# duckdb/duckdb-vss

Hardware: AMD Instinct MI355X
Metric: queries/sec at recall@10, 10M×768 FLOAT top-10; index build rows/sec (higher is better)
Workload: dtype f32

## Files before the change

### duckdb-vss_amd/__init__.py

```python
import ctypes as C
import os
import subprocess

import numpy as np

HERE = os.path.dirname(os.path.abspath(__file__))
ROOT = os.path.dirname(HERE)
LIB_PATH = os.environ.get("VSS_LIBRARY") or os.path.join(HERE, "libvssgpu.so")
CSRC = os.path.join(HERE, "csrc")

METRICS = {"l2sq": 0, "cosine": 1, "ip": 2}
FUNCTIONS = {"array_distance": 0, "array_cosine_distance": 1, "array_negative_inner_product": 2}
FREE_KEY = np.iinfo(np.int64).max

HIPCC_FLAGS = ["--offload-arch=gfx950", "-O3", "-std=c++17", "-ffp-contract=off", "-fPIC", "-Wno-int-to-pointer-cast"]


TRANSLATION_UNITS = ["vss_engine.hip", "vss_exchange.hip", "kernels_l2sq.hip", "kernels_cosine.hip", "kernels_ip.hip"]


def build_library(force=False, extra_flags=(), out=None):
    out = out or os.path.join(HERE, "libvssgpu.so")
    srcs = [os.path.join(CSRC, f) for f in sorted(os.listdir(CSRC))]
    srcs.append(os.path.join(ROOT, "include", "vssgpu.h"))
# ... 34 lines not shown
    "vss_set_build_reorder": (_int, [_vp, _int]),
    "vss_set_option": (_int, [_vp, C.c_char_p, _i64]),
    "vss_search": (_int, [_vp, _vp, _u64, _u64, _vp, _vp]),
    "vss_search_batch": (_int, [_vp, _vp, _u64, _u64, _u64, _vp, _vp, _vp]),
    "vss_search_batch_device": (_int, [_vp, _vp, _u64, _u64, _u64, _vp, _vp, _vp]),
    "vss_search_batch_filtered": (_int, [_vp, _vp, _u64, _u64, _u64, _vp, _u64, _vp, _vp, _vp]),
    "vss_search_batch_filtered_device": (_int, [_vp, _vp, _u64, _u64, _u64, _vp, _u64, _vp, _vp, _vp]),
    "vss_search_batch_device_begin": (_int, [_vp, _int, _vp, _u64, _u64, _u64, _vp, _vp, _vp]),
    "vss_search_multi_device_begin": (_int, [_vp, _int, _u64, _vp, _u64, _u64, _u64, _vp, _vp, _vp]),
    "vss_search_batch_end": (_int, [_vp, _int]),
    "vss_search_exact_batch": (_int, [_vp, _vp, _u64, _u64, _vp, _vp, _vp]),
    "vss_search_exact_batch_device": (_int, [_vp, _vp, _u64, _u64, _vp, _vp, _vp]),
    "vss_last_search_stats": (_int, [_vp, _vp]),
    "vss_last_search_shape": (_int, [_vp, _vp]),
    "vss_last_search_prescore": (_int, [_vp, _vp]),
    "vss_last_search_query_stats": (_int, [_vp, _vp, _u64]),
    "vss_timing": (_int, [_vp, _vp, _int]),
    "vss_build_work": (_int, [_vp, _vp]),
    "vss_remove_batch": (_int, [_vp, _vp, _u64, _vp]),
    "vss_compact": (_int, [_vp]),
    "vss_compact_ex": (_int, [_vp, _int, _vp]),
    "vss_size": (_u64, [_vp]),
    "vss_nodes": (_u64, [_vp]),
    "vss_build_progress": (_int, [_vp, _vp, _vp]),
    "vss_capacity": (_u64, [_vp]),
    "vss_max_level": (_u64, [_vp]),
    "vss_memory_usage": (_u64, [_vp]),
    "vss_dimensions": (_u64, [_vp]),
    "vss_metric": (_int, [_vp]),
    "vss_level_stats": (_int, [_vp, _u64, _vp]),
# ... 207 lines not shown
    def last_search_stats(self):
        out = np.zeros(4, dtype=np.uint64)
        self._check(self.lib.vss_last_search_stats(self.h, _p(out)))
        return out

    def last_search_shape(self):
        out = np.zeros(8, dtype=np.uint32)
        self._check(self.lib.vss_last_search_shape(self.h, _p(out)))
        return out

    def last_search_prescore(self):
        out = np.zeros(4, dtype=np.uint64)
        self._check(self.lib.vss_last_search_prescore(self.h, _p(out)))
        return out

    def timing(self, reset=False):
        out = np.zeros(6, dtype=np.float64)
        self._check(self.lib.vss_timing(self.h, _p(out), int(reset)))
        return dict(search_kernel_ms=out[0], build_phase_a_ms=out[1], build_phase_b_ms=out[2], build_wall_ms=out[3],
                    build_batches=int(out[4]), build_retries=int(out[5]))

    def build_work(self):
        out = np.zeros(3, dtype=np.uint64)
        self._check(self.lib.vss_build_work(self.h, _p(out)))
        return dict(insert_distances=int(out[0]), insert_expansions=int(out[1]), link_distances=int(out[2]))

    def last_query_stats(self, nq):
        out = np.zeros((nq, 2), dtype=np.uint32)
        self._check(self.lib.vss_last_search_query_stats(self.h, _p(out), nq))
        return out
# ... 90 lines not shown
```

### duckdb-vss_amd/csrc/hnsw_kernels.h

```cpp
#pragma once
#include "wave_primitives.h"
#include "prescore_bound.h"
#include <type_traits>

namespace vss {

constexpr int64_t FREE_KEY = 0x7FFFFFFFFFFFFFFFll;

struct GraphView {
	RowSpace sp;
	uint32_t dim;
	uint32_t M, M0;
	uint32_t *links0;
	uint32_t *links_up;
	const uint32_t *upper_off;
	const int64_t *keys;
	uint32_t list_id_base;
	const unsigned long long *filter;
	uint64_t filter_bits;
	uint32_t twins;

	__device__ __forceinline__ bool admitted(uint32_t slot) const {
		const int64_t key = keys[slot];
		if (key == 0x7FFFFFFFFFFFFFFFll)
// ... 342 lines not shown
#define VSS_TRACE(sp, idx, expr)
#define VSS_TRACE_INC(sp, idx)
#endif
#ifndef VSS_WALKER_WAIT_SLEEP
#define VSS_WALKER_WAIT_SLEEP 1
#endif
#ifndef VSS_SCORER_IDLE_SLEEP
#define VSS_SCORER_IDLE_SLEEP 2
#endif
struct Mailbox {
	unsigned long long ticket;
	uint32_t done;
	uint32_t qa2_bits;
	uint32_t slots;
	uint32_t bound_bits;
	uint32_t pad[2];
};

struct PrescoreView {
	const uint32_t *codes;
	const RowCodeMeta *meta;
	unsigned long long *counters;
};
constexpr uint32_t PRESCORE_SLOTS = 16;
__host__ __device__ constexpr int prescore_claim_rows(int R) {
	return 4 * R;
}
__device__ __forceinline__ float code_to_float(uint32_t w, int k) {
	return (float)(int)(int8_t)(w >> (8 * k));
}
template <int MT, int NCH, int CR>
__device__ __forceinline__ unsigned long long prescore_codes(const RowSpace &sp, const PrescoreView &pv, uint32_t dim,
                                                             const float4 *q_lds, float qa2, const uint32_t *ids, int n,
// ... 147 lines not shown
				}
				VSS_LDS_ADD(lds_u32, done_or_scrap, cnt);
				worked = true;
				continue;
			}
		}
#endif
		const float qa2 = __uint_as_float(VSS_LDS_LOAD(lds_u32, &mb->qa2_bits));
		if constexpr (PRE) {
			if (pv->codes) {
				const float bound = __uint_as_float((uint32_t)uniform((int)VSS_LDS_LOAD(lds_u32, &mb->bound_bits)));
			if (bound < __builtin_inff()) {
					constexpr int CR = prescore_claim_rows(R);
					constexpr int SHIFT = CR == 16 ? 2 : CR == 8 ? 3 : 4;
					static_assert(CR == 16 || CR == 8 || CR == 4, "rows of codes per claim");
					unsigned long long left = prescore_codes<MT, NCH, CR>(sp, *pv, dim, q, qa2, ids + c, (int)cnt, bound, dist + c, pre_counts[1]);
					pre_counts[0] += cnt;
					while (left) {
						const int have = __popcll(left);
						if (have >= 3 && R >= 4)
							wave_distances_picked<MT, NCH, (R >= 4 ? 4 : 1)>(sp, q, qa2, ids + c, left, SHIFT, dist + c);
						else if (have >= 2)
							wave_distances_picked<MT, NCH, 2>(sp, q, qa2, ids + c, left, SHIFT, dist + c);
						else
							wave_distances_picked<MT, NCH, 1>(sp, q, qa2, ids + c, left, SHIFT, dist + c);
					}
					wave_sync();
					VSS_LDS_ADD_REL(lds_u32, done_or_scrap, cnt);
					VSS_TRACE_INC(sp, 29);
					worked = true;
					continue;
				}
// ... 21 lines not shown
constexpr uint32_t ENGINE_HEADER_BYTES = ENGINE_SCRAP_OFFSET + 64 * 8;

constexpr uint32_t POOL_SPIN_LIMIT = 1u << 26;

struct CrewBox {
	int n;
	float qa2;
	uint32_t walker;
	uint32_t on;
};
static_assert(sizeof(CrewBox) == 16 && sizeof(Mailbox) == 32, "engine LDS header layout");

template <int MT, int NCH, int R, bool PRE = false>
struct PoolScorer {
	static constexpr bool touches_rows = false, touches_lists = true, helpers_touch = false;
	Mailbox *mb;
	uint32_t *exit_flag;
	uint32_t *engine_error;
	uint32_t *walkers_left;
	uint32_t scorers;
	CrewBox *crew;
	uint32_t my_slot;
	uint32_t crew_ok;
	uint32_t no_requests;
	uint32_t touch_ok;
	uint32_t prescore_ok;
	mutable uint32_t crew_on = 0;
	mutable uint32_t level = 0;
	__device__ __forceinline__ void at_level(int l) const {
		level = (uint32_t)l;
	}

	__device__ __forceinline__ bool wants_requests() const {
		return !(crew_on && no_requests);
	}

	__device__ __forceinline__ bool latency_mode() const {
		return crew_on != 0 && touch_ok != 0;
	}
	__device__ __forceinline__ uint32_t active_walkers() const {
		const uint32_t active = (uint32_t)uniform((int)VSS_LDS_LOAD(lds_u32, walkers_left));
		return active ? active : 1u;
	}
	__device__ __forceinline__ void post(int buf, const RowSpace &sp, int n, float bound = __builtin_inff()) const {
		Mailbox *box = mb + buf;
		const uint32_t lg = 6u - sp.logG;
		const uint32_t x1 = ((uint32_t)n + (1u << lg) - 1u) >> lg, x2 = (x1 + 1u) >> 1;
		const uint32_t a = active_walkers();
		if (PRE && prescore_ok) {
			const bool filtered = bound < __builtin_inff() && a * x2 > scorers;
			VSS_LDS_STORE(lds_u32, &box->slots, a * x1 <= scorers ? 1u : a * x2 <= scorers ? 2u : filtered ? PRESCORE_SLOTS : (uint32_t)R);
			VSS_LDS_STORE(lds_u32, &box->bound_bits, __float_as_uint(filtered ? bound : __builtin_inff()));
		} else {
			VSS_LDS_STORE(lds_u32, &box->slots, a * x1 <= scorers ? 1u : a * x2 <= scorers ? 2u : (uint32_t)R);
		}
		VSS_LDS_STORE(lds_u32, &box->done, 0u);
		VSS_LDS_STORE_REL(lds_u64, &box->ticket, (unsigned long long)(uint32_t)n << 32);
		VSS_TRACE_INC(sp, 16);
		VSS_TRACE(sp, 17, (uint32_t)n);
	}
	__device__ __forceinline__ void wait(int buf, const RowSpace &sp, int n) const {
		Mailbox *box = mb + buf;
		uint32_t spins = 0;
		while (uniform((int)VSS_LDS_LOAD_ACQ(lds_u32, &box->done)) < n) {
			__builtin_amdgcn_s_sleep(VSS_WALKER_WAIT_SLEEP);
			if ((spins & 1023u) == 0) {
				VSS_TRACE(sp, 20, spins);
				VSS_TRACE(sp, 21, VSS_LDS_LOAD(lds_u32, &box->done));
			}
			if (++spins > POOL_SPIN_LIMIT || ((spins & 1023u) == 0 && uniform((int)VSS_LDS_LOAD(lds_u32, exit_flag)))) {
				if (lane_id() == 0) {
					VSS_LDS_STORE(lds_u32, exit_flag, 2u);
					__hip_atomic_store(engine_error, 1u, __ATOMIC_RELAXED, __HIP_MEMORY_SCOPE_SYSTEM);
				}
				__builtin_amdgcn_endpgm();
			}
		}
		wave_sync();
		VSS_TRACE_INC(sp, 18);
	}
	__device__ __forceinline__ void begin(int buf, const RowSpace &sp, float qa2, int n, float bound = __builtin_inff()) const {
		if (crew_ok && !crew_on && uniform((int)VSS_LDS_LOAD(lds_u32, walkers_left)) == 1) {
			crew_on = 1u;
#ifdef VSS_PHASE_TIMERS
			if (lane_id() < 3)
				reinterpret_cast<unsigned long long *>(reinterpret_cast<unsigned char *>(crew) - ENGINE_CREW_OFFSET + ENGINE_SCRAP_OFFSET)[lane_id()] = 0;
#endif
			VSS_LDS_STORE_REL(lds_u32, &crew->on, 1u);
		}
		if (crew_on) {
			if (lane_id() == 0) {
				crew->n = n;
				crew->qa2 = qa2;
				crew->walker = 2u * my_slot + (uint32_t)buf + (level << 8);
			}
			lds_barrier();
			return;
		}
		post(buf, sp, n, bound);
	}
	__device__ __forceinline__ void end(int buf, const RowSpace &sp, int n) const {
		if (crew_on)
			lds_barrier();
		else
			wait(buf, sp, n);
	}
	template <typename F>
	__device__ __forceinline__ void operator()(const WaveLds &lds, const RowSpace &sp, float qa2, int n, F before_loads
	                                           VSS_WC_ARG) const {
		if (n <= 0) {
			before_loads();
			return;
		}
		VSS_TICK(tp0);
		begin(0, sp, qa2, n);
		VSS_TICK(tpb);
		VSS_ACC(t_solo_passes, tp0, tpb);
		before_loads();
		VSS_TICK(tp1);
		end(0, sp, n);
		VSS_TICK(tp3);
		VSS_ACC(t_look, tp0, tp1);
		VSS_ACC(t_sync2, tp1, tp3);
	}
	__device__ __forceinline__ void dismiss_crew() const {
		if (lane_id() == 0)
			crew->n = -1;
		lds_barrier();
	}
};

template <int MT, bool AHEAD = false, class Scorer>
__device__ __forceinline__ uint32_t descend(const GraphView &gv, WaveLds &lds, float qa2, uint32_t closest,
                                            int begin_level, int end_level, const Scorer &score, WorkCounters &wc) {
	const int lane = lane_id();
	float closest_dist = wave_distance_one<MT>(gv.sp, lds.q, qa2, closest);
	wc.distances += 1;
	ListPrefetch below;
	int below_level = -1;
	const bool can_ahead = AHEAD && gv.M0 <= 64;
	for (int level = begin_level; level > end_level; --level) {
		bool changed;
		do {
			changed = false;
			const bool have_first = can_ahead && below.slot == closest && below_level == level;
			const int n = gather_neighbors<false>(gv, lds, closest, level, have_first, have_first ? below.masked() : EMPTY_SLOT);
			if constexpr (AHEAD)
				score.at_level(level);
			score(lds, gv.sp, qa2, n, [&] {
				if constexpr (AHEAD) {
					if (can_ahead && !(below.slot == closest && below_level == level - 1)) {
						below.slot = EMPTY_SLOT;
						below.request(gv, closest, level - 1);
						below_level = level - 1;
					}
				}
			} VSS_WC_PASS);
			wc.distances += n;
			wc.cycles += 1;
			for (int off = 0; off < n; off += 64) {
				const float d = (off + lane < n) ? lds.dist[off + lane] : __builtin_inff();
				float m = d;
				m = fminf(m, lane_xor<32>(m));
				m = fminf(m, lane_xor<16>(m));
				m = fminf(m, lane_xor<8>(m));
				m = fminf(m, lane_xor<4>(m));
				m = fminf(m, lane_xor<2>(m));
				m = fminf(m, lane_xor<1>(m));
				if (m < closest_dist) {
					const unsigned long long who = __ballot(d == m);
					closest_dist = m;
					closest = lds.ids[off + __builtin_ctzll(who)];
// ... 381 lines not shown
			have = L.first_two_unexpanded_entry(d1, s1, s2);
		} else {
			have = L.first_unexpanded_entry(d1, s1) >= 0 ? 1 : 0;
		}
		e_d = have > 0 ? d1 : __builtin_inff();
		e_s = have > 0 ? s1 : EMPTY_SLOT;
		if (!pool.wants_requests())
			return;
		if (have > 0)
			ahead.request(gv, s1, 0);
		if constexpr (PK > 1) {
			if (have > 1)
				ahead.request(gv, s2, 0);
		}
	};
	auto open_expansion = [&](uint32_t cs, int buf) -> int {
		VSS_TICK(tg0);
		uint32_t first_cells;
		const bool have_first = ahead.find(cs, first_cells);
		VSS_COUNT(t_slice, have_first ? 1u : 0u);
		lds.ids = sb.ids(buf);
		const int n = gather_neighbors<true>(gv, lds, cs, 0, have_first, first_cells);
		VSS_TICK(tg1);
		VSS_ACC(t_gather, tg0, tg1);
		if (n > 0)
			pool.begin(buf, gv.sp, qa2, n, L.size >= limit ? radius : __builtin_inff());
		VSS_TICK(tg2);
		VSS_ACC(t_solo_passes, tg1, tg2);
		return n;
	};
	auto accept = [&](int buf, int n) {
		const bool have = lane < n;
		const float d = have ? sb.dist(buf)[lane] : 0.f;
		const uint32_t id = have ? sb.ids(buf)[lane] : 0;
		const unsigned long long pass = __ballot(have && (L.size < limit || d < radius));
		L.accept(d, id, pass, radius);
	};

	int b = 0, n_cur = 0;
	for (;;) {
		if (n_cur == 0) {
			VSS_TICK(tk0);
			float cd;
			uint32_t cs;
			const int pos = L.first_unexpanded_entry(cd, cs);
			if (pos < 0)
				break;
			L.mark_expanded(pos);
			wc.cycles += 1;
			VSS_TICK(tk1);
			VSS_ACC(t_pick, tk0, tk1);
			n_cur = open_expansion(cs, b);
			if (n_cur < 0)
				return LEVEL_VISITED_OVERFLOW;
			request_ahead();
			continue;
		}
		VSS_TICK(tw0);
		pool.end(b, gv.sp, n_cur);
		VSS_TICK(tw1);
		VSS_ACC(t_sync2, tw0, tw1);
		wc.distances += n_cur;
		uint32_t next = EMPTY_SLOT;
		bool tie;
		{
			const bool have = lane < n_cur;
			const float d = have ? sb.dist(b)[lane] : 0.f;
			const uint32_t id = have ? sb.ids(b)[lane] : 0;
			const bool admitted = have && (L.size < limit || d < radius);
			float m = admitted ? d : __builtin_inff();
			m = fminf(m, lane_xor<32>(m));
			m = fminf(m, lane_xor<16>(m));
			m = fminf(m, lane_xor<8>(m));
			m = fminf(m, lane_xor<4>(m));
			m = fminf(m, lane_xor<2>(m));
			m = fminf(m, lane_xor<1>(m));
			const unsigned long long who = __ballot(admitted && !(d > m));
			const float ms = __int_as_float(uniform(__float_as_int(m)));
			tie = who && (__popcll(who) > 1 || !(__builtin_fabsf(ms) < __builtin_inff()) || ms == e_d);
			if (!tie)
				next = (who && ms < e_d) ? read_lane(id, __builtin_ctzll(who)) : e_s;
		}
		VSS_TICK(tw2);
		VSS_ACC(t_pick, tw1, tw2);
		if (tie) {
			accept(b, n_cur);
			n_cur = 0;
			VSS_TICK(tw3);
			VSS_ACC(t_accept, tw2, tw3);
			continue;
		}
		const int nb = 1 - b;
		int n_next = 0;
		if (next != EMPTY_SLOT) {
			wc.cycles += 1;
			n_next = open_expansion(next, nb);
			if (n_next < 0)
				return LEVEL_VISITED_OVERFLOW;
		}
		VSS_TICK(ta0);
		accept(b, n_cur);
		uint32_t first = EMPTY_SLOT;
		int pos;
		{
			float cd;
			uint32_t w = EMPTY_SLOT;
			pos = L.first_unexpanded_entry(cd, w);
			if (pos >= 0)
				first = w;
		}
		if (first != next) {
// ... 95 lines not shown
	float *out_d[MAX_COALESCED];
	uint32_t *out_count[MAX_COALESCED];
	uint32_t *out_stats;
	uint32_t *status;
	uint32_t *retry_hash;
	uint32_t retry_log2;
	uint32_t *global_hash;
	float *list_buf;
	uint32_t list_cap;
	uint32_t list_lds;
	float *cand_buf;
	uint32_t cand_cap;
	uint32_t visited_compact;
	unsigned long long *phase_ticks;
	PrescoreView prescore;
};

__host__ __device__ inline uint32_t align16(uint32_t x) {
	return (x + 15u) & ~15u;
}

__host__ __device__ inline uint32_t wave_lds_bytes(uint32_t hash_log2, uint32_t V, uint32_t list_cap_max,
                                                   uint32_t cand_cap, bool hash_in_lds = true) {
	uint32_t b = 0;
	if (hash_in_lds)
		b += align16((1u << hash_log2) * 4);
	b += align16(V * 16) * 2;
	b += align16(list_cap_max * 4) * 2;
	b += align16(cand_cap * 4) * 2;
	b += align16((list_cap_max + 1) * 4) * 2;
// ... 261 lines not shown
		*exit_flag = 0;
		*walkers_left = S;
		crew->n = 0, crew->qa2 = 0.f, crew->walker = 0, crew->on = 0;
		a.queue[a.queue_sel ^ 2u] = 0;
	}
	VSS_TRACE(a.gv.sp, 30, blockDim.x);
	VSS_TRACE(a.gv.sp, 31, S);
	if (lane == 0)
		smem[ENGINE_SIMD_OFFSET + wave] = (unsigned char)__builtin_amdgcn_s_getreg((1 << 11) | (4 << 6) | 4);
	if (threadIdx.x < ENGINE_BOXES) {
		boxes[threadIdx.x].ticket = 0;
		boxes[threadIdx.x].done = 0;
		boxes[threadIdx.x].qa2_bits = 0;
		boxes[threadIdx.x].slots = R;
		boxes[threadIdx.x].bound_bits = 0x7F800000u;
	}
	__syncthreads();
	constexpr bool PRE = NCH >= 2 && E >= 1 && E != LDS_LIST_E && E <= pipelined_max_regs(THREADS);

	if (wave >= S) {
		uint32_t pre_counts[2] = {0, 0};
		auto leave = [&] {
			if constexpr (PRE) {
				if (lane == 0 && pre_counts[0]) {
					atomicAdd(a.prescore.counters, (unsigned long long)pre_counts[0]);
					atomicAdd(a.prescore.counters + 1, (unsigned long long)pre_counts[1]);
				}
			}
		};
		for (;;) {
			bool worked = false;
			VSS_TRACE_INC(a.gv.sp, 24);
			for (uint32_t s = 0; s < 2 * S; ++s) {
				const unsigned long long t = VSS_LDS_LOAD(lds_u64, &boxes[s].ticket);
				if (uniform((int)((uint32_t)t < (uint32_t)(t >> 32)))) {
					const EngineSlot es =
					    engine_slot(smem, s >> 1, a.hash_log2, a.gv.sp.V, a.list_cap_max, hash_in_lds, a.stage_cap, list_cells);
					worked |= pool_score<MT, NCH, R, PRE>(&boxes[s], scrap, a.gv.sp, es.q, (s & 1) ? es.ids2 : es.ids,
					                                      (s & 1) ? es.dist2 : es.dist, &a.prescore, a.gv.dim, pre_counts);
				}
			}
// ... 14 lines not shown
	__builtin_amdgcn_s_setprio(2);
	const EngineSlot es = engine_slot(smem, wave, a.hash_log2, a.gv.sp.V, a.list_cap_max, hash_in_lds, a.stage_cap, list_cells);
	const size_t gslot = (size_t)blockIdx.x * S + wave;
	WaveLds lds;
	bind_visited(lds.visited, hash_in_lds ? es.hash : a.global_hash + (gslot << a.hash_log2), a.hash_log2);
	if constexpr (E == MAX_LIST_REGS) {
		if (a.visited_compact)
			bind_visited_compact(lds.visited, a.visited_compact);
	}
	lds.q = es.q, lds.ids = es.ids, lds.dist = es.dist;
	lds.q2 = nullptr, lds.kept_s = nullptr, lds.kept_d = nullptr;
	lds.cand_d = nullptr, lds.cand_s = nullptr;
	lds.touch_lines = a.touch_lines & TOUCH_LISTS;
	PoolScorer<MT, NCH, R, PRE> score {&boxes[2 * wave], exit_flag, a.engine_error, walkers_left, (blockDim.x >> 6) - S, crew, wave,
	                                   ((a.crew & CREW_ON) && !a.spec_active) ? 1u : 0u, (a.crew & CREW_NO_REQUESTS) ? 1u : 0u,
	                                   (a.crew & CREW_TOUCH) ? 1u : 0u, (PRE && a.prescore.codes) ? 1u : 0u};
	const SpecBuffers sb {es.ids, es.ids2, es.dist, es.dist2};
	CandQueue cq;
	cq.bind(a.cand_buf + gslot * 2 * a.cand_cap, reinterpret_cast<uint32_t *>(a.cand_buf + gslot * 2 * a.cand_cap) + a.cand_cap,
	        (int)a.cand_cap);
	typename std::conditional<E == LDS_LIST_E, LdsList,
	                          typename std::conditional<E == 0, MemList, WaveList<(E == 0 || E == LDS_LIST_E ? 1 : E)>>::type>::type L;
	if constexpr (E == 0)
		L.bind(a.list_buf + gslot * 2 * a.list_cap, reinterpret_cast<uint32_t *>(a.list_buf + gslot * 2 * a.list_cap) + a.list_cap);
	if constexpr (E == LDS_LIST_E)
		L.bind(es.list_d, es.list_s, es.list_tops);
	const int limit = a.ef > a.k ? a.ef : a.k;

	constexpr bool CAN_MOVE = E == MAX_LIST_REGS;
	if constexpr (CAN_MOVE) {
		if (a.retry_hash && hash_in_lds && es.stage_d) {
// ... 601 lines not shown
```

### duckdb-vss_amd/csrc/prescore_bound.h

```cpp
#pragma once
#include <math.h>
#include <stdint.h>

#if defined(__HIPCC__) || defined(__CUDACC__)
#define VSS_PRESCORE_HD __host__ __device__
#else
#define VSS_PRESCORE_HD
#endif

namespace vss {

struct RowCodeMeta {
	float scale;
	float err;
	float norm;
	uint32_t spare;
};

constexpr float PRESCORE_NO_BOUND = -INFINITY;

VSS_PRESCORE_HD inline double prescore_slack(uint32_t dim) {
	return ((double)dim + 64.0) * (1.0 / 2097152.0);
}

// ... 22 lines not shown
	} else {
		if (!(fabsf(t) < INFINITY))
			return PRESCORE_NO_BOUND;
		const double ub = scale * (double)t + qn * E;
		const double qr = qn * rn;
		if (metric == 1)
			lb = 1.0 - ub / qr - slack;
		else
			lb = 1.0 - ub - slack * qr - 0x1p-22 * (1.0 + qr);
	}
	if (!(lb == lb))
		return PRESCORE_NO_BOUND;
	return prescore_round_down(lb);
}

}
```

### duckdb-vss_amd/csrc/vss_engine.hip

```cpp
#include <hip/hip_runtime.h>

#include <algorithm>
#include <atomic>
#include <chrono>
#include <cmath>
#include <cstdarg>
#include <cstdio>
#include <cstdlib>
#include <cstring>
#include <condition_variable>
#include <mutex>
#include <shared_mutex>
#include <string>
#include <thread>
#include <vector>

#define VSS_ENGINE_TU
#include "../../include/vssgpu.h"
#include "launchers.h"
#include "host_logic.h"
#include "row_codes.h"

using namespace vss;
using namespace vss::host;
// ... 137 lines not shown
		uint32_t queue_sel = 0;
		size_t h_cap = 0;
		hipEvent_t ev0 = nullptr, ev1 = nullptr;
		bool pending = false;
		bool direct_io = false;
		SearchArgs args;
		uint64_t nq = 0, limit = 0, list_cap = 0;
		uint32_t bump = 0;
		uint32_t min_hash_log2 = 0;
		uint32_t shape[8] = {0, 0, 0, 0, 0, 0, 0, 0};
		bool first_pass = true;
		double kernel_ms = 0;
		uint64_t stats[4] = {0, 0, 0, 0};
		DevBuf<unsigned long long> d_prescore;
		unsigned long long *h_prescore = nullptr;
		unsigned long long prescore_base[2] = {0, 0};
		bool prescore_first = false, prescore_used = false;
	};
	static constexpr int EXPLICIT_CTX = 4, MAX_CTX = 12;
	SearchCtx ctx[MAX_CTX];
	std::mutex lease_mu;
	std::condition_variable lease_cv;
	int lease_context() {
		std::unique_lock<std::mutex> lk(lease_mu);
		for (;;) {
			for (int i = EXPLICIT_CTX; i != MAX_CTX; ++i)
				if (!ctx[i].leased) {
					ctx[i].leased = true;
					return i;
				}
			lease_cv.wait(lk);
// ... 4 lines not shown
			std::lock_guard<std::mutex> lk(lease_mu);
			ctx[i].leased = false;
		}
		lease_cv.notify_one();
	}
	std::mutex ctx0_mu;
	std::mutex exact_mu;

	uint32_t search_prescore = 1;
	DevBuf<uint32_t> d_codes;
	DevBuf<RowCodeMeta> d_code_meta;
	StaleSlots codes_stale;
	std::mutex codes_mu;
	uint64_t codes_refused_capacity = 0;
	uint64_t last_prescore[4] = {0, 0, 0, 0};
	bool codes_wanted() const {
		const uint32_t nch = (G == 64 && V % 64 == 0 && !force_looping) ? V / 64 : 0;
		return search_prescore && (nch == 2 || nch == 3 || nch == 4 || nch == 6);
	}
	void free_codes() {
		d_codes.free(), d_code_meta.free();
		codes_stale.clear();
		codes_refused_capacity = 0;
	}
	bool ensure_codes(hipStream_t s, bool may_allocate) {
		if (!codes_wanted() || !capacity)
			return false;
		std::lock_guard<std::mutex> lk(codes_mu);
		if (d_codes.n < capacity * V || d_code_meta.n < capacity) {
			if (!may_allocate || codes_refused_capacity == capacity)
// ... 705 lines not shown
		a.touch_lines = shape.touch_lines;
		a.crew = shape.crew ? (CREW_ON | ((search_touch_lists && list_cap_max() <= 64) ? CREW_TOUCH : 0u) | search_crew_tune) : 0u;
		a.pipelined = (can_pipeline && (wide_list || c.limit <= 64u * PIPELINED_MAX_REGS)) ? 1u : 0u;
		a.prescore = PrescoreView {nullptr, nullptr, nullptr};
		bool codes_ready = false;
		const bool wide_limit = c.limit > 64u * PIPELINED_MAX_REGS;
		if (a.pipelined && !solo && !c.direct_io && (search_prescore == 2 || !wide_limit)) {
			try {
				codes_ready = ensure_codes(c.stream, false);
			} catch (const HipError &) {
				(void)hipGetLastError();
			}
		}
		if (codes_ready) {
			if (!c.d_prescore.p) {
				c.d_prescore.ensure(2, 0, c.stream, 0);
				HIP_TRY(hipHostMalloc((void **)&c.h_prescore, 2 * sizeof(unsigned long long), hipHostMallocDefault));
				c.h_prescore[0] = c.h_prescore[1] = 0;
				c.prescore_base[0] = c.prescore_base[1] = 0;
			}
			a.prescore = PrescoreView {d_codes.p, d_code_meta.p, c.d_prescore.p};
			c.prescore_used = true;
		}
		if (c.first_pass)
			c.prescore_first = a.prescore.codes != nullptr;
		a.global_hash = nullptr;
		if (!hash_in_lds) {
			c.d_global_hash.ensure(((uint64_t)grid * S) << a.hash_log2, 0, c.stream);
			a.global_hash = c.d_global_hash.p;
		}
		a.retry_hash = nullptr, a.retry_log2 = 0;
		if (retry_want_log2 && c.d_retry_hash.try_ensure(((uint64_t)grid * S) << retry_want_log2))
			a.retry_hash = c.d_retry_hash.p, a.retry_log2 = retry_want_log2;
		a.list_cap = (uint32_t)c.list_cap;
		a.list_buf = nullptr;
		if (c.list_cap && !list_in_lds) {
			c.d_list_buf.ensure((uint64_t)grid * S * 2 * c.list_cap, 0, c.stream);
			a.list_buf = c.d_list_buf.p;
// ... 46 lines not shown
		else
			HIP_TRY(hipEventRecord(c.ev0, c.stream));
		if (solo)
			launch_by_metric<SearchArgs>(launch_search_solo<0>, launch_search_solo<1>, launch_search_solo<2>, a, cfg);
		else
			launch_by_metric<SearchArgs>(launch_search<0>, launch_search<1>, launch_search<2>, a, cfg);
		if (c.flag_wait)
			c.flag_target = (c.unsynced ? c.flag_target : 0u) + n;
		else
			HIP_TRY(hipEventRecord(c.ev1, c.stream));
		if (!c.direct_io) {
			HIP_TRY(hipMemcpyAsync(c.h_status, c.d_status.p, c.nq * 4, hipMemcpyDeviceToHost, c.stream));
			HIP_TRY(hipMemcpyAsync(c.h_stats, c.d_stats.p, c.nq * 8, hipMemcpyDeviceToHost, c.stream));
		}
		if (a.prescore.codes)
			HIP_TRY(hipMemcpyAsync(c.h_prescore, c.d_prescore.p, 2 * sizeof(unsigned long long), hipMemcpyDeviceToHost, c.stream));
	}

	bool search_gating = true;
	void wait_for_drain_of_previous_launch(int slot);
	bool probe_flag_wait = true;
	bool search_touch_rows = true, search_touch_lists = true;
	uint32_t search_touch_max_queries = 256;
	bool search_team = true;
	bool search_crew = true;
	uint32_t search_crew_tune = 0;
	bool search_pipelined = true;
	bool search_wide_lists = true;
	uint32_t search_list_lds = 1;

	int search_begin(int slot, const float *d_queries, uint32_t q_stride, uint64_t nq, uint64_t k, uint64_t ef,
// ... 198 lines not shown
			c.d_work.ensure(c.nq, 0, c.stream);
			HIP_TRY(hipMemcpyAsync(c.d_work.p, work.data(), work.size() * 4, hipMemcpyHostToDevice, c.stream));
			HIP_TRY(hipStreamSynchronize(c.stream));
			c.args.work = c.d_work.p;
			launch_search_kernel(c, (uint32_t)work.size());
		}
		for (uint64_t i = 0; i != c.nq; ++i) {
			c.stats[0] += c.h_stats[2 * i];
			c.stats[1] += c.h_stats[2 * i + 1];
		}
		{
			std::lock_guard<std::mutex> lk(stats_mu);
			std::memcpy(last_stats, c.stats, sizeof last_stats);
			std::memcpy(last_shape, c.shape, sizeof last_shape);
			last_prescore[0] = c.prescore_first ? 1 : 0;
			last_prescore[1] = last_prescore[2] = 0;
			if (c.prescore_used) {
				last_prescore[1] = c.h_prescore[0] - c.prescore_base[0];
				last_prescore[2] = c.h_prescore[1] - c.prescore_base[1];
				c.prescore_base[0] = c.h_prescore[0], c.prescore_base[1] = c.h_prescore[1];
			}
			last_prescore[3] = d_codes.n * sizeof(uint32_t) + d_code_meta.n * sizeof(RowCodeMeta);
			timing[0] = c.kernel_ms;
			if (keep_query_stats)
				last_query_stats.assign(c.h_stats, c.h_stats + 2 * c.nq);
		}
		return VSS_OK;
	}

	int search_launch(int slot, const float *d_queries, uint32_t q_stride, uint64_t nq, uint64_t k, uint64_t ef,
	                  int64_t *d_keys_out, float *d_dist_out, uint32_t *d_count_out, bool keep_query_stats,
	                  const uint64_t *d_filter = nullptr, uint64_t filter_bits = 0, bool direct_io = false) {
		std::unique_lock<std::mutex> lk0(ctx0_mu, std::defer_lock);
		if (slot == 0)
			lk0.lock();
		int rc = search_begin(slot, d_queries, q_stride, nq, k, ef, d_keys_out, d_dist_out, d_count_out, d_filter,
// ... 824 lines not shown
     "one expansion of look-ahead while at most this many walkers of a workgroup still run (0 = off)"},
    {"search.gating", 0, 1, [](vss_index *h, int64_t v) { h->search_gating = v != 0; },
     "a launch is issued when its predecessor on the device starts to drain"},
    {"search.list_lds", 0, 2, [](vss_index *h, int64_t v) { h->search_list_lds = (uint32_t)v; },
     "candidate lists of limits 513-4096 in LDS: 0 never (HBM), 1 when the workgroup keeps its walkers, 2 whenever one walker fits"},
    {"search.prescore", 0, 2,
     [](vss_index *h, int64_t v) {
	     h->search_prescore = (uint32_t)v;
	     if (!h->search_prescore)
		     h->free_codes();
	     else if (h->stream)
		     h->refresh_codes();
     },
     "scoring waves reject rows on exact bounds from 8-bit row codes before reading their f32 components: 0 never, 1 at limits of "
     "at most 256, 2 in every pipelined launch"},
};
const char *set_option_checked(vss_index *h, const char *name, int64_t value) {
	for (const OptionRule &r : OPTION_RULES) {
		if (std::strcmp(r.name, name))
			continue;
		if (value < r.lo || value > r.hi)
			return "value out of range";
		if (!std::strcmp(name, "search.visited_cells_per_limit") && value != 0 && value < 4)
			return "value out of range";
		const uint32_t waves = !std::strcmp(name, "search.waves") ? (uint32_t)value : h->search_waves;
		const uint32_t walkers = !std::strcmp(name, "search.walkers") ? (uint32_t)value : h->search_walkers;
		if (walkers && walkers >= waves)
			return "at least one scoring wave must remain";
		r.apply(h, value);
		return nullptr;
// ... 42 lines not shown
		return VSS_ERROR;
	}
	std::memset(h->h_debug, 0, 128 * sizeof(uint32_t));
#endif
	hipDeviceProp_t prop;
	if (hipGetDeviceProperties(&prop, device) == hipSuccess && prop.multiProcessorCount > 0)
		h->n_cus = (uint32_t)prop.multiProcessorCount;
	static const struct { const char *env, *option; } ENV_OPTIONS[] = {
	    {"VSS_SEARCH_WAVES", "search.waves"}, {"VSS_SEARCH_WALKERS", "search.walkers"}, {"VSS_SEARCH_SPEC", "search.lookahead"},
	    {"VSS_SEARCH_SOLO", "search.solo"}, {"VSS_SEARCH_SOLO_MAX", "search.solo_max_queries"}, {"VSS_SEARCH_TEAM", "search.team"},
	    {"VSS_SEARCH_CREW", "search.crew"}, {"VSS_SEARCH_PIPELINED", "search.pipelined"},
	    {"VSS_SEARCH_WIDE_LISTS", "search.wide_lists"}, {"VSS_VISITED_COMPACT", "search.visited_compact"},
	    {"VSS_SEARCH_RETRY_IN_PLACE", "search.retry_in_place"}, {"VSS_HASH_LDS_MAX_LOG2", "search.visited_lds_log2_max"},
	    {"VSS_VISITED_PER_LIMIT", "search.visited_cells_per_limit"}, {"VSS_PROBE_FLAG_WAIT", "search.probe_flag_wait"},
	    {"VSS_SEARCH_LIST_LDS", "search.list_lds"}, {"VSS_SEARCH_PRESCORE", "search.prescore"},
	};
	for (const auto &e : ENV_OPTIONS)
		if (const char *t = getenv(e.env)) {
			if (const char *why = set_option_checked(h, e.option, (int64_t)atoll(t)))
				fprintf(stderr, "vssgpu: %s=%s ignored (%s: %s)\n", e.env, t, e.option, why);
		}
	if (const char *t = getenv("VSS_SEARCH_REG_QUEUE"))
		h->search_reg_queue = atoi(t) != 0;
	if (const char *t = getenv("VSS_SEARCH_REG_QUEUE_MAX"))
		h->reg_queue_max_limit = (uint32_t)std::max(0, std::min(64 * MAX_LIST_REGS, atoi(t)));
	if (const char *t = getenv("VSS_FORCE_LOOPING"))
		h->force_looping = atoi(t) != 0;
	if (const char *t = getenv("VSS_EXACT_PROBE"))
		h->exact_probe = (uint32_t)atoi(t);
	if (const char *t = getenv("VSS_EXACT_KERNEL"))
// ... 225 lines not shown
	VSS_SHARED(h, {
		std::lock_guard<std::mutex> lk(h->stats_mu);
		std::memcpy(out4, h->last_stats, sizeof h->last_stats);
		return VSS_OK;
	})
}

int vss_last_search_prescore(vss_index *h, uint64_t *out4) {
	VSS_SHARED(h, {
		std::lock_guard<std::mutex> lk(h->stats_mu);
		std::memcpy(out4, h->last_prescore, sizeof h->last_prescore);
		return VSS_OK;
	})
}

int vss_last_search_shape(vss_index *h, uint32_t *out8) {
	VSS_SHARED(h, {
		std::lock_guard<std::mutex> lk(h->stats_mu);
		std::memcpy(out8, h->last_shape, sizeof h->last_shape);
		return VSS_OK;
	})
}

#ifdef VSS_PHASE_TIMERS
int vss_debug_phase_ticks(vss_index *h, unsigned long long *out, uint64_t nq) {
	VSS_SHARED(h, {
		if (!h->ctx[0].d_phase.p || h->ctx[0].d_phase.n < nq * VSS_PHASE_STRIDE)
			return h->fail("no phase ticks recorded for %llu queries", (unsigned long long)nq);
		HIP_TRY(hipMemcpy(out, h->ctx[0].d_phase.p, nq * VSS_PHASE_STRIDE * 8, hipMemcpyDeviceToHost));
		return VSS_OK;
// ... 252 lines not shown
```

### include/vssgpu.h

```cpp
#ifndef VSSGPU_H
#define VSSGPU_H
#include <stdint.h>
#ifdef __cplusplus
extern "C" {
#endif

typedef struct vss_index vss_index;

enum { VSS_OK = 0, VSS_ERROR = 1 };

enum { VSS_METRIC_L2SQ = 0, VSS_METRIC_COSINE = 1, VSS_METRIC_IP = 2 };

enum { VSS_FN_ARRAY_DISTANCE = 0, VSS_FN_ARRAY_COSINE_DISTANCE = 1, VSS_FN_ARRAY_NEGATIVE_INNER_PRODUCT = 2 };

#define VSS_FREE_KEY INT64_MAX


int vss_create(uint64_t dim, int metric, uint64_t M, uint64_t M0, uint64_t ef_construction, uint64_t ef_search,
               int device, vss_index **out);
void vss_destroy(vss_index *index);
const char *vss_last_error(vss_index *index);
int vss_set_stream(vss_index *index, void *hip_stream);
int vss_synchronize(vss_index *index);

// ... 25 lines not shown
                                     const uint64_t *d_allowed, uint64_t n_bits, int64_t *d_out_rowids,
                                     float *d_out_distances, uint32_t *d_out_counts);
int vss_search_batch_device_begin(vss_index *index, int context, const float *d_queries, uint64_t n_queries, uint64_t k,
                                  uint64_t ef, int64_t *d_out_rowids, float *d_out_distances, uint32_t *d_out_counts);
int vss_search_multi_device_begin(vss_index *index, int context, uint64_t n_batches, const float *const *d_queries,
                                  uint64_t n_per_batch, uint64_t k, uint64_t ef, int64_t *const *d_out_rowids,
                                  float *const *d_out_distances, uint32_t *const *d_out_counts);
int vss_search_batch_end(vss_index *index, int context);
int vss_search_exact_batch(vss_index *index, const float *queries, uint64_t n_queries, uint64_t k,
                           int64_t *out_rowids, float *out_distances, uint32_t *out_counts);
int vss_search_exact_batch_device(vss_index *index, const float *d_queries, uint64_t n_queries, uint64_t k,
                                  int64_t *d_out_rowids, float *d_out_distances, uint32_t *d_out_counts);
int vss_last_search_stats(vss_index *index, uint64_t *out4);
int vss_last_search_shape(vss_index *index, uint32_t *out8);
int vss_last_search_prescore(vss_index *index, uint64_t *out4);
int vss_timing(vss_index *index, double *out6, int reset);
int vss_build_work(vss_index *index, uint64_t *out3);
int vss_last_search_query_stats(vss_index *index, uint32_t *out, uint64_t n_queries);


int vss_remove_batch(vss_index *index, const int64_t *rowids, uint64_t count, uint64_t *out_removed);
int vss_compact(vss_index *index);
int vss_compact_ex(vss_index *index, int reorder, int *out_reordered);

uint64_t vss_size(vss_index *index);
uint64_t vss_nodes(vss_index *index);
uint64_t vss_capacity(vss_index *index);
uint64_t vss_max_level(vss_index *index);
uint64_t vss_memory_usage(vss_index *index);
uint64_t vss_dimensions(vss_index *index);
// ... 46 lines not shown
```

Before: 1.662 million.

## Extend prescore bound to greedy descent jobs and add fresh-radius scope

Adds a scope mask for which scoring jobs carry a prescore bound from 8-bit row codes. Greedy upper-level descent jobs now pass the current closest distance as a bound, so scorer waves can reject rows before reading their f32 components. An optional scope tightens the level-0 bound to the radius expected after the pending accept, at the cost of extra wave reductions. Counters are split by job kind and exposed through a new stats call.

Result: slower. 1.489 million (-10.4%).

```diff
diff --git a/duckdb-vss_amd/__init__.py b/duckdb-vss_amd/__init__.py
--- a/duckdb-vss_amd/__init__.py
+++ b/duckdb-vss_amd/__init__.py
@@ -72,6 +72,7 @@
     "vss_last_search_stats": (_int, [_vp, _vp]),
     "vss_last_search_shape": (_int, [_vp, _vp]),
     "vss_last_search_prescore": (_int, [_vp, _vp]),
+    "vss_last_search_prescore_kinds": (_int, [_vp, _vp]),
     "vss_last_search_query_stats": (_int, [_vp, _vp, _u64]),
     "vss_timing": (_int, [_vp, _vp, _int]),
     "vss_build_work": (_int, [_vp, _vp]),
@@ -309,6 +310,11 @@
         self._check(self.lib.vss_last_search_prescore(self.h, _p(out)))
         return out
 
+    def last_search_prescore_kinds(self):
+        out = np.zeros(4, dtype=np.uint64)
+        self._check(self.lib.vss_last_search_prescore_kinds(self.h, _p(out)))
+        return out
+
     def timing(self, reset=False):
         out = np.zeros(6, dtype=np.float64)
         self._check(self.lib.vss_timing(self.h, _p(out), int(reset)))
diff --git a/duckdb-vss_amd/csrc/hnsw_kernels.h b/duckdb-vss_amd/csrc/hnsw_kernels.h
--- a/duckdb-vss_amd/csrc/hnsw_kernels.h
+++ b/duckdb-vss_amd/csrc/hnsw_kernels.h
@@ -380,9 +380,12 @@
 	uint32_t qa2_bits;
 	uint32_t slots;
 	uint32_t bound_bits;
-	uint32_t pad[2];
+	uint32_t kind;
+	uint32_t pad;
 };
 
+constexpr uint32_t PRESCORE_SCOPE_BASE = 1u, PRESCORE_SCOPE_DESCENT = 2u, PRESCORE_SCOPE_FRESH_RADIUS = 4u;
+constexpr uint32_t JOB_BASE = 0u, JOB_DESCENT = 1u;
 struct PrescoreView {
 	const uint32_t *codes;
 	const RowCodeMeta *meta;
@@ -560,8 +563,11 @@
 					constexpr int CR = prescore_claim_rows(R);
 					constexpr int SHIFT = CR == 16 ? 2 : CR == 8 ? 3 : 4;
 					static_assert(CR == 16 || CR == 8 || CR == 4, "rows of codes per claim");
-					unsigned long long left = prescore_codes<MT, NCH, CR>(sp, *pv, dim, q, qa2, ids + c, (int)cnt, bound, dist + c, pre_counts[1]);
-					pre_counts[0] += cnt;
+					const bool descent = uniform((int)VSS_LDS_LOAD(lds_u32, &mb->kind)) == (int)JOB_DESCENT;
+					uint32_t rejected = 0;
+					unsigned long long left = prescore_codes<MT, NCH, CR>(sp, *pv, dim, q, qa2, ids + c, (int)cnt, bound, dist + c, rejected);
+					pre_counts[0] += descent ? 0u : cnt, pre_counts[1] += descent ? 0u : rejected;
+					pre_counts[2] += descent ? cnt : 0u, pre_counts[3] += descent ? rejected : 0u;
 					while (left) {
 						const int have = __popcll(left);
 						if (have >= 3 && R >= 4)
@@ -613,6 +619,7 @@
 template <int MT, int NCH, int R, bool PRE = false>
 struct PoolScorer {
 	static constexpr bool touches_rows = false, touches_lists = true, helpers_touch = false;
+	static constexpr bool takes_bound = PRE;
 	Mailbox *mb;
 	uint32_t *exit_flag;
 	uint32_t *engine_error;
@@ -641,7 +648,8 @@
 		const uint32_t active = (uint32_t)uniform((int)VSS_LDS_LOAD(lds_u32, walkers_left));
 		return active ? active : 1u;
 	}
-	__device__ __forceinline__ void post(int buf, const RowSpace &sp, int n, float bound = __builtin_inff()) const {
+	__device__ __forceinline__ void post(int buf, const RowSpace &sp, int n, float bound = __builtin_inff(),
+	                                     uint32_t kind = JOB_BASE) const {
 		Mailbox *box = mb + buf;
 		const uint32_t lg = 6u - sp.logG;
 		const uint32_t x1 = ((uint32_t)n + (1u << lg) - 1u) >> lg, x2 = (x1 + 1u) >> 1;
@@ -650,6 +658,7 @@
 			const bool filtered = bound < __builtin_inff() && a * x2 > scorers;
 			VSS_LDS_STORE(lds_u32, &box->slots, a * x1 <= scorers ? 1u : a * x2 <= scorers ? 2u : filtered ? PRESCORE_SLOTS : (uint32_t)R);
 			VSS_LDS_STORE(lds_u32, &box->bound_bits, __float_as_uint(filtered ? bound : __builtin_inff()));
+			VSS_LDS_STORE(lds_u32, &box->kind, kind);
 		} else {
 			VSS_LDS_STORE(lds_u32, &box->slots, a * x1 <= scorers ? 1u : a * x2 <= scorers ? 2u : (uint32_t)R);
 		}
@@ -678,7 +687,8 @@
 		wave_sync();
 		VSS_TRACE_INC(sp, 18);
 	}
-	__device__ __forceinline__ void begin(int buf, const RowSpace &sp, float qa2, int n, float bound = __builtin_inff()) const {
+	__device__ __forceinline__ void begin(int buf, const RowSpace &sp, float qa2, int n, float bound = __builtin_inff(),
+	                                      uint32_t kind = JOB_BASE) const {
 		if (crew_ok && !crew_on && uniform((int)VSS_LDS_LOAD(lds_u32, walkers_left)) == 1) {
 			crew_on = 1u;
 #ifdef VSS_PHASE_TIMERS
@@ -696,7 +706,7 @@
 			lds_barrier();
 			return;
 		}
-		post(buf, sp, n, bound);
+		post(buf, sp, n, bound, kind);
 	}
 	__device__ __forceinline__ void end(int buf, const RowSpace &sp, int n) const {
 		if (crew_on)
@@ -707,12 +717,23 @@
 	template <typename F>
 	__device__ __forceinline__ void operator()(const WaveLds &lds, const RowSpace &sp, float qa2, int n, F before_loads
 	                                           VSS_WC_ARG) const {
+		scored(lds, sp, qa2, n, before_loads, __builtin_inff(), JOB_BASE VSS_WC_PASS);
+	}
+	template <typename F>
+	__device__ __forceinline__ void descent_job(const WaveLds &lds, const RowSpace &sp, float qa2, int n, F before_loads,
+	                                            float closest_dist VSS_WC_ARG) const {
+		scored(lds, sp, qa2, n, before_loads, (PRE && (prescore_ok & PRESCORE_SCOPE_DESCENT)) ? closest_dist : __builtin_inff(),
+		       JOB_DESCENT VSS_WC_PASS);
+	}
+	template <typename F>
+	__device__ __forceinline__ void scored(const WaveLds &lds, const RowSpace &sp, float qa2, int n, F before_loads, float bound,
+	                                       uint32_t kind VSS_WC_ARG) const {
 		if (n <= 0) {
 			before_loads();
 			return;
 		}
 		VSS_TICK(tp0);
-		begin(0, sp, qa2, n);
+		begin(0, sp, qa2, n, bound, kind);
 		VSS_TICK(tpb);
 		VSS_ACC(t_solo_passes, tp0, tpb);
 		before_loads();
@@ -728,6 +749,11 @@
 		lds_barrier();
 	}
 };
+
+template <class Scorer, class = void>
+struct scorer_takes_bound : std::false_type {};
+template <class Scorer>
+struct scorer_takes_bound<Scorer, typename std::enable_if<Scorer::takes_bound>::type> : std::true_type {};
 
 template <int MT, bool AHEAD = false, class Scorer>
 __device__ __forceinline__ uint32_t descend(const GraphView &gv, WaveLds &lds, float qa2, uint32_t closest,
@@ -746,7 +772,7 @@
 			const int n = gather_neighbors<false>(gv, lds, closest, level, have_first, have_first ? below.masked() : EMPTY_SLOT);
 			if constexpr (AHEAD)
 				score.at_level(level);
-			score(lds, gv.sp, qa2, n, [&] {
+			auto look_below = [&] {
 				if constexpr (AHEAD) {
 					if (can_ahead && !(below.slot == closest && below_level == level - 1)) {
 						below.slot = EMPTY_SLOT;
@@ -754,7 +780,11 @@
 						below_level = level - 1;
 					}
 				}
-			} VSS_WC_PASS);
+			};
+			if constexpr (scorer_takes_bound<Scorer>::value)
+				score.descent_job(lds, gv.sp, qa2, n, look_below, closest_dist VSS_WC_PASS);
+			else
+				score(lds, gv.sp, qa2, n, look_below VSS_WC_PASS);
 			wc.distances += n;
 			wc.cycles += 1;
 			for (int off = 0; off < n; off += 64) {
@@ -1166,7 +1196,7 @@
 				ahead.request(gv, s2, 0);
 		}
 	};
-	auto open_expansion = [&](uint32_t cs, int buf) -> int {
+	auto open_expansion = [&](uint32_t cs, int buf, float bound) -> int {
 		VSS_TICK(tg0);
 		uint32_t first_cells;
 		const bool have_first = ahead.find(cs, first_cells);
@@ -1175,11 +1205,21 @@
 		const int n = gather_neighbors<true>(gv, lds, cs, 0, have_first, first_cells);
 		VSS_TICK(tg1);
 		VSS_ACC(t_gather, tg0, tg1);
-		if (n > 0)
-			pool.begin(buf, gv.sp, qa2, n, L.size >= limit ? radius : __builtin_inff());
+		if (n > 0) {
+			if constexpr (scorer_takes_bound<Pool>::value)
+				pool.begin(buf, gv.sp, qa2, n, bound);
+			else
+				pool.begin(buf, gv.sp, qa2, n);
+		}
 		VSS_TICK(tg2);
 		VSS_ACC(t_solo_passes, tg1, tg2);
 		return n;
+	};
+	auto plain_bound = [&]() -> float {
+		if constexpr (scorer_takes_bound<Pool>::value)
+			return (pool.prescore_ok & (PRESCORE_SCOPE_BASE | PRESCORE_SCOPE_FRESH_RADIUS)) && L.size >= limit ? radius : __builtin_inff();
+		else
+			return __builtin_inff();
 	};
 	auto accept = [&](int buf, int n) {
 		const bool have = lane < n;
@@ -1202,7 +1242,7 @@
 			wc.cycles += 1;
 			VSS_TICK(tk1);
 			VSS_ACC(t_pick, tk0, tk1);
-			n_cur = open_expansion(cs, b);
+			n_cur = open_expansion(cs, b, plain_bound());
 			if (n_cur < 0)
 				return LEVEL_VISITED_OVERFLOW;
 			request_ahead();
@@ -1215,6 +1255,7 @@
 		wc.distances += n_cur;
 		uint32_t next = EMPTY_SLOT;
 		bool tie;
+		float bound_next;
 		{
 			const bool have = lane < n_cur;
 			const float d = have ? sb.dist(b)[lane] : 0.f;
@@ -1232,6 +1273,38 @@
 			tie = who && (__popcll(who) > 1 || !(__builtin_fabsf(ms) < __builtin_inff()) || ms == e_d);
 			if (!tie)
 				next = (who && ms < e_d) ? read_lane(id, __builtin_ctzll(who)) : e_s;
+			bound_next = plain_bound();
+			if constexpr (scorer_takes_bound<Pool>::value) {
+				if ((pool.prescore_ok & PRESCORE_SCOPE_FRESH_RADIUS) && !tie && next != EMPTY_SLOT) {
+					const bool full = L.size >= limit;
+					const int f = full ? __popcll(__ballot(admitted)) : n_cur;
+					const bool unusable = __ballot(have && prescore_fresh_unusable(d, full)) != 0ull;
+					if (!unusable && f > 0 && L.size + f >= limit) {
+						float a_pick = radius, pick;
+						if (full) {
+							float mx = admitted ? d : -__builtin_inff();
+							mx = fmaxf(mx, lane_xor<32>(mx));
+							mx = fmaxf(mx, lane_xor<16>(mx));
+							mx = fmaxf(mx, lane_xor<8>(mx));
+							mx = fmaxf(mx, lane_xor<4>(mx));
+							mx = fmaxf(mx, lane_xor<2>(mx));
+							mx = fmaxf(mx, lane_xor<1>(mx));
+							pick = __int_as_float(uniform(__float_as_int(mx)));
+							if (f < limit) {
+								uint32_t unused;
+								L.get(limit - 1 - f, a_pick, unused);
+							}
+						} else {
+							int rank = 0;
+							for (int j = 0; j < n_cur; ++j)
+								rank += prescore_fresh_before(read_lane(d, j), j, d, lane) ? 1 : 0;
+							const unsigned long long kth = __ballot(have && rank == limit - L.size - 1);
+							pick = kth ? read_lane(d, __builtin_ctzll(kth)) : __builtin_inff();
+						}
+						bound_next = prescore_radius_after_accept(L.size, limit, f, a_pick, pick, bound_next);
+					}
+				}
+			}
 		}
 		VSS_TICK(tw2);
 		VSS_ACC(t_pick, tw1, tw2);
@@ -1246,7 +1319,7 @@
 		int n_next = 0;
 		if (next != EMPTY_SLOT) {
 			wc.cycles += 1;
-			n_next = open_expansion(next, nb);
+			n_next = open_expansion(next, nb, bound_next);
 			if (n_next < 0)
 				return LEVEL_VISITED_OVERFLOW;
 		}
@@ -1372,6 +1445,7 @@
 	uint32_t visited_compact;
 	unsigned long long *phase_ticks;
 	PrescoreView prescore;
+	uint32_t prescore_scope;
 };
 
 __host__ __device__ inline uint32_t align16(uint32_t x) {
@@ -1663,17 +1737,20 @@
 		boxes[threadIdx.x].qa2_bits = 0;
 		boxes[threadIdx.x].slots = R;
 		boxes[threadIdx.x].bound_bits = 0x7F800000u;
+		boxes[threadIdx.x].kind = JOB_BASE;
 	}
 	__syncthreads();
 	constexpr bool PRE = NCH >= 2 && E >= 1 && E != LDS_LIST_E && E <= pipelined_max_regs(THREADS);
 
 	if (wave >= S) {
-		uint32_t pre_counts[2] = {0, 0};
+		uint32_t pre_counts[4] = {0, 0, 0, 0};
 		auto leave = [&] {
 			if constexpr (PRE) {
-				if (lane == 0 && pre_counts[0]) {
+				if (lane == 0 && (pre_counts[0] | pre_counts[2])) {
 					atomicAdd(a.prescore.counters, (unsigned long long)pre_counts[0]);
 					atomicAdd(a.prescore.counters + 1, (unsigned long long)pre_counts[1]);
+					atomicAdd(a.prescore.counters + 2, (unsigned long long)pre_counts[2]);
+					atomicAdd(a.prescore.counters + 3, (unsigned long long)pre_counts[3]);
 				}
 			}
 		};
@@ -1718,7 +1795,7 @@
 	lds.touch_lines = a.touch_lines & TOUCH_LISTS;
 	PoolScorer<MT, NCH, R, PRE> score {&boxes[2 * wave], exit_flag, a.engine_error, walkers_left, (blockDim.x >> 6) - S, crew, wave,
 	                                   ((a.crew & CREW_ON) && !a.spec_active) ? 1u : 0u, (a.crew & CREW_NO_REQUESTS) ? 1u : 0u,
-	                                   (a.crew & CREW_TOUCH) ? 1u : 0u, (PRE && a.prescore.codes) ? 1u : 0u};
+	                                   (a.crew & CREW_TOUCH) ? 1u : 0u, (PRE && a.prescore.codes) ? a.prescore_scope : 0u};
 	const SpecBuffers sb {es.ids, es.ids2, es.dist, es.dist2};
 	CandQueue cq;
 	cq.bind(a.cand_buf + gslot * 2 * a.cand_cap, reinterpret_cast<uint32_t *>(a.cand_buf + gslot * 2 * a.cand_cap) + a.cand_cap,
diff --git a/duckdb-vss_amd/csrc/prescore_bound.h b/duckdb-vss_amd/csrc/prescore_bound.h
--- a/duckdb-vss_amd/csrc/prescore_bound.h
+++ b/duckdb-vss_amd/csrc/prescore_bound.h
@@ -60,4 +60,56 @@
 	return prescore_round_down(lb);
 }
 
+
+VSS_PRESCORE_HD inline bool prescore_fresh_before(float dj, int j, float di, int i) {
+	return dj < di || (dj == di && j < i);
 }
+VSS_PRESCORE_HD inline bool prescore_fresh_unusable(float d, bool full) {
+	return !(d > -INFINITY) || (!full && !(d < INFINITY));
+}
+VSS_PRESCORE_HD inline float prescore_radius_after_accept(int size, int limit, int f, float a_pick, float fresh_pick,
+                                                          float old_bound) {
+	if (f <= 0)
+		return old_bound;
+	if (size + f < limit)
+		return INFINITY;
+	const bool full = size >= limit;
+	const bool use_a = full ? f < limit : size > 0;
+	const float u = use_a && a_pick > fresh_pick ? a_pick : fresh_pick;
+	if (!(u == u))
+		return old_bound;
+	return u < old_bound ? u : old_bound;
+}
+VSS_PRESCORE_HD inline float prescore_radius_after_accept_serial(const float *a, int size, int limit, const float *fresh,
+                                                                 int n) {
+	const bool full = size >= limit;
+	const float radius = size > 0 ? a[size - 1] : INFINITY;
+	const float old_bound = full ? radius : INFINITY;
+	int f = 0;
+	bool unusable = false;
+	for (int i = 0; i < n; ++i) {
+		unusable = unusable || prescore_fresh_unusable(fresh[i], full);
+		f += (!full || fresh[i] < radius) ? 1 : 0;
+	}
+	if (unusable || f == 0 || size + f < limit)
+		return unusable || f == 0 ? old_bound : INFINITY;
+	float pick = -INFINITY;
+	if (full) {
+		for (int i = 0; i < n; ++i)
+			if (fresh[i] < radius && fresh[i] > pick)
+				pick = fresh[i];
+	} else {
+		const int k = limit - size;
+		for (int i = 0; i < n; ++i) {
+			int rank = 0;
+			for (int j = 0; j < n; ++j)
+				rank += prescore_fresh_before(fresh[j], j, fresh[i], i) ? 1 : 0;
+			if (rank == k - 1)
+				pick = fresh[i];
+		}
+	}
+	const float a_pick = full ? (f < limit ? a[limit - 1 - f] : 0.f) : radius;
+	return prescore_radius_after_accept(size, limit, f, a_pick, pick, old_bound);
+}
+
+}
diff --git a/duckdb-vss_amd/csrc/vss_engine.hip b/duckdb-vss_amd/csrc/vss_engine.hip
--- a/duckdb-vss_amd/csrc/vss_engine.hip
+++ b/duckdb-vss_amd/csrc/vss_engine.hip
@@ -175,7 +175,7 @@
 		uint64_t stats[4] = {0, 0, 0, 0};
 		DevBuf<unsigned long long> d_prescore;
 		unsigned long long *h_prescore = nullptr;
-		unsigned long long prescore_base[2] = {0, 0};
+		unsigned long long prescore_base[4] = {0, 0, 0, 0};
 		bool prescore_first = false, prescore_used = false;
 	};
 	static constexpr int EXPLICIT_CTX = 4, MAX_CTX = 12;
@@ -210,6 +210,8 @@
 	std::mutex codes_mu;
 	uint64_t codes_refused_capacity = 0;
 	uint64_t last_prescore[4] = {0, 0, 0, 0};
+	uint64_t last_prescore_kinds[4] = {0, 0, 0, 0};
+	uint32_t search_prescore_scope = PRESCORE_SCOPE_BASE | PRESCORE_SCOPE_DESCENT;
 	bool codes_wanted() const {
 		const uint32_t nch = (G == 64 && V % 64 == 0 && !force_looping) ? V / 64 : 0;
 		return search_prescore && (nch == 2 || nch == 3 || nch == 4 || nch == 6);
@@ -945,14 +947,15 @@
 		}
 		if (codes_ready) {
 			if (!c.d_prescore.p) {
-				c.d_prescore.ensure(2, 0, c.stream, 0);
-				HIP_TRY(hipHostMalloc((void **)&c.h_prescore, 2 * sizeof(unsigned long long), hipHostMallocDefault));
-				c.h_prescore[0] = c.h_prescore[1] = 0;
-				c.prescore_base[0] = c.prescore_base[1] = 0;
+				c.d_prescore.ensure(4, 0, c.stream, 0);
+				HIP_TRY(hipHostMalloc((void **)&c.h_prescore, 4 * sizeof(unsigned long long), hipHostMallocDefault));
+				for (int i = 0; i < 4; ++i)
+					c.h_prescore[i] = c.prescore_base[i] = 0;
 			}
 			a.prescore = PrescoreView {d_codes.p, d_code_meta.p, c.d_prescore.p};
 			c.prescore_used = true;
 		}
+		a.prescore_scope = search_prescore_scope;
 		if (c.first_pass)
 			c.prescore_first = a.prescore.codes != nullptr;
 		a.global_hash = nullptr;
@@ -1029,7 +1032,7 @@
 			HIP_TRY(hipMemcpyAsync(c.h_stats, c.d_stats.p, c.nq * 8, hipMemcpyDeviceToHost, c.stream));
 		}
 		if (a.prescore.codes)
-			HIP_TRY(hipMemcpyAsync(c.h_prescore, c.d_prescore.p, 2 * sizeof(unsigned long long), hipMemcpyDeviceToHost, c.stream));
+			HIP_TRY(hipMemcpyAsync(c.h_prescore, c.d_prescore.p, 4 * sizeof(unsigned long long), hipMemcpyDeviceToHost, c.stream));
 	}
 
 	bool search_gating = true;
@@ -1258,12 +1261,16 @@
 			std::memcpy(last_stats, c.stats, sizeof last_stats);
 			std::memcpy(last_shape, c.shape, sizeof last_shape);
 			last_prescore[0] = c.prescore_first ? 1 : 0;
-			last_prescore[1] = last_prescore[2] = 0;
+			for (int i = 0; i < 4; ++i)
+				last_prescore_kinds[i] = 0;
 			if (c.prescore_used) {
-				last_prescore[1] = c.h_prescore[0] - c.prescore_base[0];
-				last_prescore[2] = c.h_prescore[1] - c.prescore_base[1];
-				c.prescore_base[0] = c.h_prescore[0], c.prescore_base[1] = c.h_prescore[1];
-			}
+				for (int i = 0; i < 4; ++i) {
+					last_prescore_kinds[i] = c.h_prescore[i] - c.prescore_base[i];
+					c.prescore_base[i] = c.h_prescore[i];
+				}
+			}
+			last_prescore[1] = last_prescore_kinds[0] + last_prescore_kinds[2];
+			last_prescore[2] = last_prescore_kinds[1] + last_prescore_kinds[3];
 			last_prescore[3] = d_codes.n * sizeof(uint32_t) + d_code_meta.n * sizeof(RowCodeMeta);
 			timing[0] = c.kernel_ms;
 			if (keep_query_stats)
@@ -2118,6 +2125,9 @@
      },
      "scoring waves reject rows on exact bounds from 8-bit row codes before reading their f32 components: 0 never, 1 at limits of "
      "at most 256, 2 in every pipelined launch"},
+    {"search.prescore_scope", 0, 7, [](vss_index *h, int64_t v) { h->search_prescore_scope = (uint32_t)v; },
+     "which jobs carry a pre-scoring bound, a bit mask: 1 level-0 jobs with the radius at hand-over, 2 the greedy descent's jobs, "
+     "4 level-0 jobs with the radius after the pending accept"},
 };
 const char *set_option_checked(vss_index *h, const char *name, int64_t value) {
 	for (const OptionRule &r : OPTION_RULES) {
@@ -2190,6 +2200,7 @@
 	    {"VSS_SEARCH_RETRY_IN_PLACE", "search.retry_in_place"}, {"VSS_HASH_LDS_MAX_LOG2", "search.visited_lds_log2_max"},
 	    {"VSS_VISITED_PER_LIMIT", "search.visited_cells_per_limit"}, {"VSS_PROBE_FLAG_WAIT", "search.probe_flag_wait"},
 	    {"VSS_SEARCH_LIST_LDS", "search.list_lds"}, {"VSS_SEARCH_PRESCORE", "search.prescore"},
+	    {"VSS_SEARCH_PRESCORE_SCOPE", "search.prescore_scope"},
 	};
 	for (const auto &e : ENV_OPTIONS)
 		if (const char *t = getenv(e.env)) {
@@ -2445,6 +2456,14 @@
 	})
 }
 
+int vss_last_search_prescore_kinds(vss_index *h, uint64_t *out4) {
+	VSS_SHARED(h, {
+		std::lock_guard<std::mutex> lk(h->stats_mu);
+		std::memcpy(out4, h->last_prescore_kinds, sizeof h->last_prescore_kinds);
+		return VSS_OK;
+	})
+}
+
 int vss_last_search_shape(vss_index *h, uint32_t *out8) {
 	VSS_SHARED(h, {
 		std::lock_guard<std::mutex> lk(h->stats_mu);
diff --git a/include/vssgpu.h b/include/vssgpu.h
--- a/include/vssgpu.h
+++ b/include/vssgpu.h
@@ -63,6 +63,7 @@
 int vss_last_search_stats(vss_index *index, uint64_t *out4);
 int vss_last_search_shape(vss_index *index, uint32_t *out8);
 int vss_last_search_prescore(vss_index *index, uint64_t *out4);
+int vss_last_search_prescore_kinds(vss_index *index, uint64_t *out4);
 int vss_timing(vss_index *index, double *out6, int reset);
 int vss_build_work(vss_index *index, uint64_t *out3);
 int vss_last_search_query_stats(vss_index *index, uint32_t *out, uint64_t n_queries);
```
